# refresh-bio/vclust

Hardware: AMD Instinct MI355X
Metric: genome pairs/sec through prefilter+align (ani.tsv) (higher is better)
Workload: dtype u64

## Files before the change

include/vclust_gpu.h:

```cpp
#ifndef VCLUST_GPU_H
#define VCLUST_GPU_H

#include <stdint.h>

#ifdef __cplusplus
extern "C" {
#endif

enum {
    VG_OK = 0, VG_EINVAL = -1, VG_EIO = -2, VG_ENODEV = -3, VG_EHIP = -4, VG_ENOMEM = -5,
    VG_EOVERFLOW = -6
};

const char* vg_version(void);
const char* vg_last_error(void);
void        vg_free(void* p);
int vg_device_count(void);
int vg_set_device(int device);
void vg_release_device_memory(void);
int vg_alloc_selftest(const int64_t* sizes, int n_sizes, int cycles);
int vg_copy(void* dst, const void* src, int64_t bytes, int to_host);

typedef struct vg_genomes vg_genomes;

// ... 15 lines not shown

int vg_kmer_shared(vg_genomes* g, int k, double fraction, int shard, int n_shards,
                   uint32_t min_shared, int64_t* set_sizes, vg_pair_count** pairs,
                   int64_t* n_pairs);
int vg_kmer_shared_new(vg_genomes* g, int n_db, int k, double fraction, uint32_t min_shared, int64_t* set_sizes,
                       vg_pair_count** pairs, int64_t* n_pairs);
void vg_set_new_path(int mode);
typedef struct {
    int accepted; int64_t P; int n_passes;
    int levels, total_bits, B1, B2;
    int st_tiles; int64_t n_st; int u_st, g_st;
    int tile32k, narrow, short_rec;
} vg_kmer_geometry_info;
int vg_kmer_geometry(const vg_genomes* g, int k, double fraction, int shard, int n_shards, vg_kmer_geometry_info* info);
int vg_kmer_geometry_at(int64_t padded_positions, int k, vg_kmer_geometry_info* info);
int vg_kmer_set(vg_genomes* g, int idx, int k, double fraction, uint64_t** out, int64_t* n_out);

int vg_write_fltr(const vg_genomes* g, int k, double fraction, int min_kmers, double min_ident,
                  int max_seqs, const int64_t* set_sizes, const vg_pair_count* pairs,
                  int64_t n_pairs, const char* out_path);

int vg_filter_pairs(int k, int min_kmers, double min_ident, const int64_t* set_sizes, int64_t n_genomes,
                    const vg_pair_count* pairs, int64_t n_pairs, vg_pair_count** out, int64_t* n_out);

typedef struct {
    int    k;
    int    min_kmers;
    double min_ident;
    int    batch_size;
    double kmers_fraction;
// ... 195 lines not shown
```

vclust_amd/_lib.py:

```python
import ctypes as C
import pathlib

PKG_DIR = pathlib.Path(__file__).resolve().parent
LIB_PATH = PKG_DIR / 'libvclust_gpu.so'


class VclustGpuError(RuntimeError):
    def __init__(self, code, msg):
        super().__init__(f'libvclust_gpu error {code}: {msg}')
        self.code = code


class PairCount(C.Structure):
    _fields_ = [('a', C.c_uint32), ('b', C.c_uint32), ('shared', C.c_uint32)]


class Task(C.Structure):
    _fields_ = [('q', C.c_uint32), ('r', C.c_uint32)]


class PairStat(C.Structure):
    _fields_ = [('n_match', C.c_uint32), ('aln_len', C.c_uint32), ('n_regions', C.c_uint32)]


# ... 96 lines not shown
    'vg_genomes_load': (C.c_int, [P(C.c_char_p), C.c_int, C.c_int, C.c_int, P(C.c_void_p)]),
    'vg_genomes_load_db_new': (C.c_int, [P(C.c_char_p), C.c_int, P(C.c_char_p), C.c_int, C.c_int, C.c_int, P(C.c_void_p), P(C.c_int)]),
    'vg_genomes_from_codes': (C.c_int, [C.c_void_p, C.c_void_p, C.c_int, P(C.c_char_p), P(C.c_void_p)]),
    'vg_genomes_free': (None, [C.c_void_p]),
    'vg_genomes_count': (C.c_int, [C.c_void_p]),
    'vg_genomes_total_len': (C.c_int64, [C.c_void_p]),
    'vg_genomes_lengths': (C.c_int, [C.c_void_p, P(C.c_int64)]),
    'vg_genomes_name': (C.c_char_p, [C.c_void_p, C.c_int]),
    'vg_genomes_codes': (C.c_int, [C.c_void_p, C.c_int, C.c_void_p]),
    'vg_genomes_to_device': (C.c_int, [C.c_void_p]),
    'vg_kmer_shared': (C.c_int, [C.c_void_p, C.c_int, C.c_double, C.c_int, C.c_int, C.c_uint32,
                                 P(C.c_int64), P(P(PairCount)), P(C.c_int64)]),
    'vg_kmer_shared_new': (C.c_int, [C.c_void_p, C.c_int, C.c_int, C.c_double, C.c_uint32, P(C.c_int64), P(P(PairCount)), P(C.c_int64)]),
    'vg_kmer_geometry': (C.c_int, [C.c_void_p, C.c_int, C.c_double, C.c_int, C.c_int, P(KmerGeometry)]),
    'vg_kmer_geometry_at': (C.c_int, [C.c_int64, C.c_int, P(KmerGeometry)]),
    'vg_kmer_set': (C.c_int, [C.c_void_p, C.c_int, C.c_int, C.c_double, P(P(C.c_uint64)), P(C.c_int64)]),
    'vg_filter_pairs': (C.c_int, [C.c_int, C.c_int, C.c_double, C.POINTER(C.c_int64), C.c_int64, C.POINTER(PairCount), C.c_int64,
                                  C.POINTER(C.POINTER(PairCount)), C.POINTER(C.c_int64)]),
    'vg_write_fltr': (C.c_int, [C.c_void_p, C.c_int, C.c_double, C.c_int, C.c_double, C.c_int,
                                P(C.c_int64), P(PairCount), C.c_int64, C.c_char_p]),
    'vg_prefilter': (C.c_int, [P(C.c_char_p), C.c_int, C.c_char_p, P(PrefilterParams)]),
    'vg_prefilter_new': (C.c_int, [P(C.c_char_p), C.c_int, P(C.c_char_p), C.c_int, C.c_char_p, P(PrefilterParams)]),
    'vg_set_process_ends_after_call': (None, [C.c_int]),
    'vg_set_lz_fit': (None, [P(LzFit)]),
    'vg_lz_align': (C.c_int, [C.c_void_p, P(Task), C.c_int64, P(LzParams), P(PairStat),
                              P(P(Region)), P(C.c_int64)]),
    'vg_align_order': (C.c_int, [C.c_void_p, P(C.c_int32)]),
    'vg_read_filter': (C.c_int, [C.c_void_p, C.c_char_p, C.c_double, P(P(PairCount)), P(C.c_int64)]),
    'vg_align_tasks': (C.c_int, [C.c_void_p, P(PairCount), C.c_int64, P(P(Task)), P(C.c_int64)]),
    'vg_lz_prepare': (C.c_int, [C.c_void_p, P(PairCount), C.c_int64, P(LzParams)]),
# ... 98 lines not shown
```

vclust_amd/api.py:

```python
import ctypes as C
import inspect
import os

import numpy as np

from . import _lib
from ._lib import (CLUSTER_ALGORITHMS, LINKAGE_ALGORITHMS, AlignParams, ClusterStats, DedupStats, KernelTime, LinkageStats, LzParams, PairCount, PairStat,
                   PrefilterParams, Region, Task, check)

ALIGN_FIELDS = ['qidx', 'ridx', 'query', 'reference', 'tani', 'gani', 'ani', 'qcov', 'rcov',
                'num_alns', 'len_ratio', 'qlen', 'rlen', 'nt_match', 'nt_mismatch']

PAIR_DTYPE = np.dtype([('a', '<u4'), ('b', '<u4'), ('shared', '<u4')])
TASK_DTYPE = np.dtype([('q', '<u4'), ('r', '<u4')])
STAT_DTYPE = np.dtype([('n_match', '<u4'), ('aln_len', '<u4'), ('n_regions', '<u4')])
REGION_DTYPE = np.dtype([('task', '<u4'), ('qstart', '<i4'), ('qend', '<i4'), ('rstart', '<i4'),
                         ('rend', '<i4'), ('n_match', '<i4')])
LINKAGE_DTYPE = np.dtype([('node_a', '<i8'), ('node_b', '<i8'), ('similarity', '<f8'), ('size', '<i8'), ('object_a', '<i4'),
                          ('object_b', '<i4')])

from .stages import DEFAULT_LZ


def version():
# ... 418 lines not shown

def set_placement_trials(n):
    _lib.load().vg_set_placement_trials(int(n))


def set_new_path(mode):
    _lib.load().vg_set_new_path(int(mode))


def kmer_geometry_at(padded_positions, k=25):
    info = _lib.KmerGeometry()
    check(_lib.load().vg_kmer_geometry_at(int(padded_positions), int(k), C.byref(info)))
    return {name: int(getattr(info, name)) for name, _ in info._fields_}


def release_device_memory():
    _lib.load().vg_release_device_memory()


def profile_enable(on=True):
    _lib.load().vg_profile_enable(int(bool(on)))


def profile_reset():
    _lib.load().vg_profile_reset()


def profile_get():
    lib = _lib.load()
    arr = (KernelTime * 64)()
# ... 4 lines not shown
```

vclust_amd/csrc/vg_prefilter.hip:

```cpp
#include "vg_common.h"
#include <functional>
#include <map>
#include <mutex>
#include <optional>
#include <rocprim/rocprim.hpp>
#include <algorithm>
#include <cmath>
#include <cstring>

namespace {

constexpr uint64_t SENT = ~0ULL;
constexpr uint32_t SCRAMBLE32 = 0x9E3779B1u;
__host__ __device__ __forceinline__ uint64_t scramble_key(uint64_t cano, int k) {
    const uint32_t L = (uint32_t)cano & ((1u << k) - 1u);
    const uint32_t H = (uint32_t)(cano >> k);
    return ((uint64_t)(H ^ ((L * SCRAMBLE32) >> (32 - k))) << k) | L;
}
__host__ __device__ __forceinline__ uint64_t unscramble_key(uint64_t key, int k) { return scramble_key(key, k); }
constexpr uint32_t DUP_BIT = 0x80000000u;

__device__ __forceinline__ uint64_t mix64(uint64_t x) {
    x ^= x >> 33; x *= 0xff51afd7ed558ccdULL; x ^= x >> 33;
    x *= 0xc4ceb9fe1a85ec53ULL; x ^= x >> 33; return x;
}

__device__ __forceinline__ uint64_t rev2(uint64_t x) {
    x = __brevll(x);
    return ((x >> 1) & 0x5555555555555555ULL) | ((x & 0x5555555555555555ULL) << 1);
}

struct kmer_args {
    const uint32_t* planes; const uint32_t* nmask; const uint32_t* blk2g; const int64_t* base_off; const int64_t* len;
    int64_t P; int k; int use_frac; uint64_t frac_thr; uint32_t shard, n_shards; int blk_shift;
    uint32_t dig_lo, dig_n;
// ... 319 lines not shown
            const bool has_next = kk[j + 1] == key;
            const bool dup = has_prev && gg[j - 1] == g;
            gen[i] = g | (dup ? DUP_BIT : 0u);
            if (dup) { atomicAdd(&dup_per_genome[g], 1); continue; }
            if (!has_prev && !has_next) continue;
            if (!has_prev) continue;
            rowinfo[p] = (uint32_t)run_lower(keys, i, key) + 1u;
        }
    }
}

__global__ void __launch_bounds__(256)
k_group_runs(const uint64_t* __restrict__ keys, const uint32_t* __restrict__ pos, const uint32_t* __restrict__ blk2g, int blk_shift,
             int64_t n, int low_bit, uint32_t* __restrict__ gen, uint32_t* __restrict__ rowinfo,
             compact_map M, int* __restrict__ dup_per_genome, int64_t* __restrict__ long_list, unsigned int* __restrict__ n_long,
             unsigned int long_cap) {
    __shared__ uint64_t sk[GS_TILE + GS_HALO + 1];
    __shared__ uint32_t sp[GS_TILE + GS_HALO + 1];
    __shared__ unsigned long long sh[(GS_TILE + GS_HALO + 1) / 64 + 2];
    constexpr int SLOTS = (GS_TILE + GS_HALO + 1 + 255) / 256 * 256;
    const int64_t n_tiles = (n + GS_TILE - 1) / GS_TILE;
    for (int64_t tile = blockIdx.x; tile < n_tiles; tile += gridDim.x) {
        const int64_t t0 = tile * GS_TILE;
        const int m = (int)min<int64_t>((int64_t)GS_TILE + GS_HALO + 1, n - t0 + 1);
        __syncthreads();
        for (int j = threadIdx.x; j < m; j += blockDim.x) {
            const int64_t g = t0 - 1 + j;
            const uint32_t p = g >= 0 ? pos[g] : 0u;
            sk[j] = g >= 0 ? keys[g] : ~0ULL;
            sp[j] = p;
        }
// ... 20 lines not shown
                if (j == gs) { const unsigned int o = atomicAdd(n_long, 1u); if (o < long_cap) long_list[o] = t0 - 1 + gs; }
                continue;
            }
            const uint64_t key = sk[j];
            int lt = 0, eq_before = 0, eq_after = 0, prev_eq = -1;
            for (int t = gs; t < ge; ++t) {
                const uint64_t kt = sk[t];
                lt += kt < key;
                if (kt == key) { if (t < j) { ++eq_before; prev_eq = t; } else if (t > j) ++eq_after; }
            }
            const uint32_t rl = (uint32_t)(eq_before + eq_after + 1);
            if (rl < 2) continue;
            const int64_t rs = t0 - 1 + gs + lt;
            const uint32_t pj = sp[j];
            const uint32_t g = M.cblk ? genome_of_compact(M, pj) : blk2g[pj >> blk_shift];
            bool dup = false;
            if (prev_eq >= 0) { const uint32_t pq = sp[prev_eq]; dup = (M.cblk ? genome_of_compact(M, pq) : blk2g[pq >> blk_shift]) == g; }
            gen[rs + eq_before] = g | (dup ? DUP_BIT : 0u);
            if (dup) { atomicAdd(&dup_per_genome[g], 1); continue; }
            if (eq_before == 0) continue;
            const uint32_t p = sp[j];
            rowinfo[p] = (uint32_t)rs + 1u;
        }
    }
}

__global__ void __launch_bounds__(256)
k_long_groups(const uint64_t* __restrict__ keys, const uint32_t* __restrict__ pos, const uint32_t* __restrict__ blk2g, int blk_shift,
              int64_t n, int low_bit, const int64_t* __restrict__ long_list, uint32_t* __restrict__ gen, uint32_t* __restrict__ rowinfo,
              compact_map M, int* __restrict__ dup_per_genome, unsigned int* __restrict__ need_full_sort) {
    __shared__ int64_t s_end;
    const int64_t gs = long_list[blockIdx.x];
    const uint64_t key0 = keys[gs]; const uint64_t pre = key0 >> low_bit;
    if (threadIdx.x == 0) s_end = n;
    __syncthreads();
    bool same = true;
    for (int64_t base = gs; base < n; base += blockDim.x) {
// ... 35 lines not shown
            uint32_t old = atomicCAS(&hk[h], HT_EMPTY, b);
            if (old == HT_EMPTY) { atomicAdd(n_used, 1u); atomicAdd(&hc[h], 1u); return true; }
            if (old == b) { atomicAdd(&hc[h], 1u); return true; }
        }
        h = (h + 1) & (HT_SIZE - 1);
    }
    return false;
}

template <int HT_BITS, bool COMPACT = false>
__global__ void __launch_bounds__(256)
k_spgemm(const uint32_t* __restrict__ rowinfo, const uint32_t* __restrict__ gen, uint64_t n_gen,
         const int64_t* __restrict__ base_off, const int64_t* __restrict__ len, const uint32_t* __restrict__ wave_base,
         int n_genomes, uint32_t min_emit, const uint32_t* __restrict__ row_list, int n_rows,
         vg_pair_count* __restrict__ out, unsigned long long* __restrict__ out_cursor,
         unsigned long long out_cap, uint32_t* __restrict__ overflow_rows, uint32_t* __restrict__ n_overflow) {
    constexpr int HT_SIZE = 1 << HT_BITS;
    constexpr int ROWS_PER_TRIP = 16;
    __shared__ uint32_t hk[HT_SIZE];
    __shared__ uint32_t hc[HT_SIZE];
    constexpr int LQC = COMPACT ? 64 : LQ_CAP;
    __shared__ uint32_t lq[LQC];
    __shared__ uint32_t rq[COMPACT ? 64 * ROWS_PER_TRIP : 1];
    __shared__ uint32_t s_used, s_lq, s_fail, s_first;
    const int per_xcd = (n_rows + 7) / 8;
    for (int k = (int)(blockIdx.x / 8); k < per_xcd; k += (int)(gridDim.x / 8)) {
    const int row = (int)(blockIdx.x % 8) * per_xcd + k;
    if (row >= n_rows) break;
    const uint32_t a = row_list ? row_list[row] : (uint32_t)row;
    __syncthreads();
    for (int i = threadIdx.x; i < HT_SIZE; i += blockDim.x) { hk[i] = HT_EMPTY; hc[i] = 0; }
    if (threadIdx.x == 0) { s_used = 0; s_lq = 0; s_fail = 0; }
    __syncthreads();
    const int64_t p0 = wave_base ? (int64_t)wave_base[base_off[a] >> 6] : base_off[a];
    const int64_t L = wave_base ? (int64_t)wave_base[base_off[a + 1] >> 6] - p0 : len[a];
    auto walk = [&](uint32_t rs) {
        bool done = false;
        uint32_t e = 0;
        for (; e < (uint32_t)LONG_RUN && !done; e += 4) {
            uint32_t g4[4];
            __builtin_memcpy(g4, gen + (size_t)rs + e, 16);
#pragma unroll
            for (int j = 0; j < 4; ++j) {
                if (done) continue;
                const uint32_t g = g4[j];
                if (g & DUP_BIT) continue;
                if (g >= a) { done = true; continue; }
                if (!ht_add<HT_BITS>(hk, hc, g, &s_used)) s_fail = 1;
            }
        }
        if (!done) {
            const uint32_t slot = atomicAdd(&s_lq, 1u);
            if (slot < LQC) lq[slot] = rs + e;
            else for (uint64_t x = (uint64_t)rs + e; x < n_gen; ++x) {
                const uint32_t g = gen[x];
                if (g & DUP_BIT) continue;
                if (g >= a) break;
                if (!ht_add<HT_BITS>(hk, hc, g, &s_used)) s_fail = 1;
            }
        }
    };
    for (int64_t base = 0; base < L; base += (int64_t)blockDim.x * ROWS_PER_TRIP) {
        uint32_t rr4[ROWS_PER_TRIP];
#pragma unroll
        for (int u = 0; u < ROWS_PER_TRIP; ++u) {
            const int64_t i = base + (int64_t)u * blockDim.x + threadIdx.x;
            rr4[u] = (i < L) ? rowinfo[p0 + i] : 0u;
        }
        if (COMPACT) {
            const int lane = threadIdx.x & 63;
            uint32_t nq = 0;
#pragma unroll
            for (int u = 0; u < ROWS_PER_TRIP; ++u) {
                const bool nz = rr4[u] != 0u;
                const unsigned long long b = __ballot(nz);
                if (nz) rq[nq + (uint32_t)__popcll(b & ((1ULL << lane) - 1ULL))] = rr4[u];
                nq += (uint32_t)__popcll(b);
            }
            __syncthreads();
            for (uint32_t qi = (uint32_t)lane; qi < nq; qi += 64u) walk(rq[qi] - 1u);
        } else {
#pragma unroll
        for (int u = 0; u < ROWS_PER_TRIP; ++u) {
            if (!rr4[u]) continue;
            walk(rr4[u] - 1u);
        }
        }
        __syncthreads();
        if (s_lq >= LQC / 2 || base + (int64_t)blockDim.x * ROWS_PER_TRIP >= L) {
            const uint32_t nq = s_lq < LQC ? s_lq : LQC;
            for (uint32_t qi = 0; qi < nq; ++qi) {
                for (uint64_t c0 = lq[qi]; ; c0 += blockDim.x) {
                    if (threadIdx.x == 0) s_first = 0xffffffffu;
                    __syncthreads();
                    const uint64_t x = c0 + threadIdx.x;
                    const uint32_t g = x < n_gen ? gen[x] : 0u;
                    const bool stop = x >= n_gen || (!(g & DUP_BIT) && g >= a);
                    if (stop) atomicMin(&s_first, (uint32_t)threadIdx.x);
                    __syncthreads();
                    const uint32_t f = s_first;
// ... 22 lines not shown
    __syncthreads();
    if (mine) {
        unsigned long long o = ((unsigned long long)lq[1] << 32 | lq[0]) + at;
        for (int i = threadIdx.x; i < HT_SIZE; i += blockDim.x) {
            const uint32_t b = hk[i];
            if (b != HT_EMPTY && hc[i] >= min_emit) { if (o < out_cap) { out[o].a = a; out[o].b = b; out[o].shared = hc[i]; } ++o; }
        }
    }
    }
}

__global__ void __launch_bounds__(256)
k_spgemm_dense(const uint32_t* __restrict__ rowinfo, const uint32_t* __restrict__ gen, uint64_t n_gen,
               const int64_t* __restrict__ base_off, const int64_t* __restrict__ len, const uint32_t* __restrict__ wave_base,
               int n_genomes, uint32_t min_emit, const uint32_t* __restrict__ rows, uint32_t* __restrict__ dense ,
               vg_pair_count* __restrict__ out, unsigned long long* __restrict__ out_cursor, unsigned long long out_cap) {
    const uint32_t a = rows[blockIdx.x];
    uint32_t* cnt = dense + (size_t)blockIdx.x * n_genomes;
    const int64_t p0 = wave_base ? (int64_t)wave_base[base_off[a] >> 6] : base_off[a];
    const int64_t L = wave_base ? (int64_t)wave_base[base_off[a + 1] >> 6] - p0 : len[a];
    for (int64_t i = threadIdx.x; i < L; i += blockDim.x) {
        const uint32_t r = rowinfo[p0 + i];
        if (!r) continue;
        for (uint64_t x = (uint64_t)r - 1; x < n_gen; ++x) {
            const uint32_t g = gen[x];
            if (g & DUP_BIT) continue;
            if (g >= a) break;
            atomicAdd(&cnt[g], 1u);
        }
    }
    __syncthreads();
    for (uint32_t b = threadIdx.x; b < a; b += blockDim.x) {
        uint32_t c = cnt[b];
        if (c >= min_emit && c > 0) {
            unsigned long long o = atomicAdd(out_cursor, 1ULL);
            if (o < out_cap) { out[o].a = a; out[o].b = b; out[o].shared = c; }
        }
    }
// ... 830 lines not shown
        uint32_t acc = run;
        for (int u = 0; u < n_u; ++u) { const uint32_t t = tab[(size_t)u * nb2 + c]; tab[(size_t)u * nb2 + c] = acc; acc += t; }
        run += tot[v];
    }
    if (b1 == nb1 - 1 && threadIdx.x == 0) boff[(size_t)nb1 * nb2] = off1[nb1];
}

constexpr int BK_PER = BK_CAP / BK_THREADS;
constexpr int BK_MAXBIN = 768;
template <bool NARROW, int THREADS, int SUBBITS>
__global__ void __launch_bounds__(THREADS)
k_bucket_runs(const uint32_t* __restrict__ rec, int stride ,
              const uint32_t* __restrict__ boff, int64_t n_buckets, int pbits, const uint32_t* __restrict__ blk2g, int blk_shift,
              uint32_t* __restrict__ gen, uint32_t* __restrict__ rowinfo, compact_map M, int* __restrict__ dup_per_genome,
              const uint32_t* __restrict__ bucket_list ,
              uint32_t* __restrict__ over_list, unsigned int* __restrict__ n_over) {
    constexpr int BK_SUB = 1 << SUBBITS, CAP = THREADS * BK_PER;
    static_assert(CAP <= 8192 && BK_MAXBIN <= 1024, "slot | rank << 13 of the run members");
    __shared__ uint32_t s_big;
    __shared__ uint64_t sk[CAP];
    __shared__ uint32_t sp[NARROW ? 1 : CAP];
    __shared__ uint32_t sgen[CAP];
    __shared__ uint32_t cnt[BK_SUB + 1], start[BK_SUB + 1];
    __shared__ uint32_t s_wave[THREADS / 64];
    const int lane = threadIdx.x & 63, wv = threadIdx.x >> 6;
    for (int64_t it = blockIdx.x; it < n_buckets; it += gridDim.x) {
        const int64_t bk = bucket_list ? (int64_t)bucket_list[it] : it;
        const uint32_t b0 = boff[bk], b1 = boff[bk + 1];
        const uint32_t n_u = b1 - b0;
        if (n_u <= 1) continue;
        if (n_u > (uint32_t)CAP) { if (threadIdx.x == 0) over_list[atomicAdd(n_over, 1u)] = (uint32_t)bk; continue; }
        const int n = (int)n_u;
// ... 85 lines not shown
                for (uint32_t t = s0; t < s1; ++t) {
                    const uint64_t kt = sk[t];
                    lt += kt < kq;
                    if (kt == kq) { ++eq; before += sp[t] < pq; }
                }
            }
            if (eq < 2) continue;
            const uint32_t g = M.cblk ? genome_of_compact(M, pq) : blk2g[pq >> blk_shift];
            sgen[s0 + lt + before] = g;
            if (before) { at[q] = (s0 + lt + before) | (before << 13); gq[q] = g; }
        }
        lds_sync();
#pragma unroll
        for (int q = 0; q < BK_PER; ++q) {
            if (at[q] == 0xffffffffu) continue;
            const uint32_t slot = at[q] & 0x1fffu, g = gq[q];
            if ((sgen[slot - 1] & ~DUP_BIT) == g) { sgen[slot] = g | DUP_BIT; atomicAdd(&dup_per_genome[g], 1); continue; }
            rowinfo[pj[q]] = b0 + (slot - (at[q] >> 13)) + 1u;
        }
        lds_sync();
        for (uint32_t i = 4u * threadIdx.x; i < (uint32_t)n; i += 4u * THREADS) {
            if (i + 4 <= (uint32_t)n) { const uint4 v = make_uint4(sgen[i], sgen[i + 1], sgen[i + 2], sgen[i + 3]); __builtin_memcpy(gen + b0 + i, &v, 16); }
            else for (uint32_t j = i; j < (uint32_t)n; ++j) gen[b0 + j] = sgen[j];
        }
    }
}

constexpr int BB_THREADS = 1024;
constexpr int BB_DIGITS = 12;
__device__ __forceinline__ uint32_t bb_scan_incl_add(uint32_t v, uint32_t* s_w, uint32_t* carry) {
    const int lane = threadIdx.x & 63, wv = threadIdx.x >> 6;
    uint32_t x = v;
#pragma unroll
// ... 18 lines not shown
    __syncthreads();
    uint32_t base = *carry, tot = *carry;
#pragma unroll
    for (int i = 0; i < BB_THREADS / 64; ++i) { const uint32_t t = s_w[i]; if (i < wv) base = max(base, t); tot = max(tot, t); }
    const uint32_t r = max(base, x);
    __syncthreads();
    if (threadIdx.x == 0) *carry = tot;
    __syncthreads();
    return r;
}
__global__ void __launch_bounds__(BB_THREADS)
k_bucket_big(const uint32_t* __restrict__ rec, int stride, const uint32_t* __restrict__ boff, const uint32_t* __restrict__ list,
             const uint64_t* __restrict__ soff , int pbits,
             uint64_t* __restrict__ kA, uint32_t* __restrict__ pA, uint64_t* __restrict__ kB, uint32_t* __restrict__ pB,
             const uint32_t* __restrict__ blk2g, int blk_shift, uint32_t* __restrict__ gen, uint32_t* __restrict__ rowinfo,
             compact_map M, int* __restrict__ dup_per_genome) {
    __shared__ uint32_t hist[BB_DIGITS][256];
    __shared__ uint32_t gbase[256];
    __shared__ uint32_t wcnt[BB_THREADS / 64][256];
    __shared__ uint32_t s_w[BB_THREADS / 64];
    __shared__ uint32_t s_carry_a, s_carry_b;
    const int lane = threadIdx.x & 63, wv = threadIdx.x >> 6;
    const uint32_t bk = list[blockIdx.x];
    const uint32_t b0 = boff[bk];
    const uint32_t n = boff[bk + 1] - b0;
    uint64_t* k0 = kA + soff[blockIdx.x]; uint32_t* p0 = pA + soff[blockIdx.x];
    uint64_t* k1 = kB + soff[blockIdx.x]; uint32_t* p1 = pB + soff[blockIdx.x];
    for (int i = threadIdx.x; i < BB_DIGITS * 256; i += BB_THREADS) (&hist[0][0])[i] = 0;
    __syncthreads();
    for (uint32_t i = threadIdx.x; i < n; i += BB_THREADS) {
        const uint32_t* r = rec + (uint64_t)(b0 + i) * stride;
// ... 68 lines not shown
        }
        const uint32_t s_incl = bb_scan_incl_add(nd, s_w, &s_carry_a);
        const uint32_t rs = bb_scan_incl_max(hd, s_w, &s_carry_b);
        if (i < n) { S[2 * (uint64_t)i] = s_incl | (nd ? 0u : 0x80000000u); S[2 * (uint64_t)i + 1] = rs; }
    }
    __threadfence_block();
    __syncthreads();
    for (uint32_t i = threadIdx.x; i < n; i += BB_THREADS) {
        const uint32_t sv = S[2 * (uint64_t)i], rs = S[2 * (uint64_t)i + 1];
        const uint32_t pos = p0[i];
        const uint32_t g = M.cblk ? genome_of_compact(M, pos) : blk2g[pos >> blk_shift];
        if (sv & 0x80000000u) { atomicAdd(&dup_per_genome[g], 1); continue; }
        const uint32_t base = rs ? (S[2 * (uint64_t)(rs - 1)] & 0x7fffffffu) : 0u;
        const uint32_t rank = (sv & 0x7fffffffu) - 1u - base;
        gen[(uint64_t)b0 + rs + rank] = g;
        if (rank > 0) rowinfo[pos] = b0 + rs + 1u;
    }
}

__global__ void k_bucket_sizes(const uint32_t* __restrict__ boff, const uint32_t* __restrict__ list, int64_t n, uint32_t* __restrict__ sizes) {
    for (int64_t i = (int64_t)blockIdx.x * blockDim.x + threadIdx.x; i < n; i += (int64_t)gridDim.x * blockDim.x) sizes[i] = boff[list[i] + 1] - boff[list[i]];
}

struct max_op { __device__ __host__ uint32_t operator()(uint32_t a, uint32_t b) const { return a > b ? a : b; } };

}

static int g_force_subshards = 0;
static const char* pf_switch(const char* name) { const char* e = vg_dev_getenv(name); return e ? e : ""; }
static const struct {
    bool radix = !strcmp(pf_switch("VG_INDEX_PATH"), "radix");
    bool long_rec = !strcmp(pf_switch("VG_LEVEL1_RECORDS"), "long");
    bool old_scatter = !strcmp(pf_switch("VG_DENSE_SCATTER"), "staged");
    bool range_dense = !strcmp(pf_switch("VG_RANGE_SCATTER"), "dense");
    bool staged2 = !strcmp(pf_switch("VG_LEVEL2_SCATTER"), "staged");
    bool scan_each = !strcmp(pf_switch("VG_SUBSHARD_SCAN"), "each");
    int subshards = atoi(pf_switch("VG_SUBSHARDS"));
    int placement_trials = atoi(pf_switch("VG_PLACEMENT_TRIALS"));
    double workspace_gb = [] { const char* e = getenv("VG_WORKSPACE_GB"); const double v = e ? atof(e) : 0.0; return v > 0.01 ? v : 8.0; }();
} g_sw{};
template <class F> static void with_k(bool k25, F f) { if (k25) f(std::integral_constant<int, 25>{}); else f(std::integral_constant<int, 0>{}); }
constexpr double SUB_PASS_KMERS = 3.6e9, SUB_PASS_START = 3.9e9;

static bool range_shards(int64_t P, double fraction, int n_shards) {
    return n_shards > 1 && n_shards <= 256 && !(fraction < 1.0) && P < (1LL << 32);
}
static bool range_shards(const vg_genomes* g, double fraction, int n_shards) { return range_shards(g->padded_total(), fraction, n_shards); }
static kmer_args shard_kmer_args(int64_t P, int align_shift, int k, double fraction, int shard, int n_shards) {
    const int use_frac = fraction < 1.0;
    kmer_args A{ nullptr, nullptr, nullptr, nullptr, nullptr, P, k, use_frac,
                 use_frac ? (uint64_t)std::ldexp(fraction, 64) : ~0ULL, (uint32_t)shard, (uint32_t)n_shards, align_shift, 0u, 1u << DIG_BITS, 1u << DIG_BITS };
    if (range_shards(P, fraction, n_shards)) {
        A.dig_max = (uint32_t)(((1u << DIG_BITS) + (uint32_t)n_shards - 1u) / (uint32_t)n_shards);
        const uint32_t lo = (uint32_t)(((uint64_t)shard << DIG_BITS) / (uint64_t)n_shards), hi = (uint32_t)(((uint64_t)(shard + 1) << DIG_BITS) / (uint64_t)n_shards);
        A.shard = 0; A.n_shards = 1; A.dig_lo = lo; A.dig_n = hi - lo;
// ... 243 lines not shown
        if (mine.m_off.empty()) { mine.m_off.assign((size_t)W + 1, 0); mine.t_off.assign((size_t)W + 1, 0); }
        if (status != VG_OK) vg_set_error("%s", err.c_str());
        const vg_xpart parts[2] = { { mine.mask.p, mine.m_off.data(), wave_mask, m_roff.data() }, { mine.T.p, mine.t_off.data(), T1s, t_roff.data() } };
        xs->alltoallv(status, parts, 2);
    }
    if (W_total > 0) hipLaunchKernelGGL(k_mask_popc, dim3(grid_for(W_total)), dim3(256), 0, s, (const unsigned long long*)wave_mask, W_total, wave_cnt);
    VG_HIP(hipStreamSynchronize(s));
}

struct kmer_index {
    sorted_index si;
    dbuf<uint32_t> arena;
    dbuf<uint32_t> rowinfo, gen; dbuf<int> d_dups;
    std::vector<int> kept, dups;
    int64_t nv = 0, n_rows_info = 0;
    bool compact_rows = false, rows_from_map = false;
    const uint32_t* wbase = nullptr;
};
struct bucket_geometry {
    bool range, big_buckets, narrow, tile32k, short_rec;
    int total_bits, B1, B2, levels, bin_lo, nb1g, nb1, nb2, st_tiles, n_slabs; int64_t n_st, nbk;
    lvl2_tab L2;
};
static bool bucket_geometry_for(int k, bool dense, const kmer_args& A, int64_t n_src, bucket_geometry& G) {
    G.range = dense && A.dig_n < (1u << DIG_BITS);
    if (g_sw.radix || n_src < (1 << 16) || n_src >= (1LL << 32)) return false;
    const int64_t n_expect = dense && !G.range ? n_src / std::max<uint32_t>(1u, A.n_shards) : n_src;
    if (!bucket_digits(n_expect, &G.total_bits, &G.B1, &G.B2)) return false;
    G.big_buckets = (n_expect >> G.total_bits) > 1024; G.levels = G.total_bits > 11 ? 2 : 1;
    if (G.range && G.B1 > DIG_BITS) return false;
// ... 143 lines not shown
        }
    }
    VG_HIP(hipStreamSynchronize(s));
    vg_host_mark("buckets: level 2 done");
    vg_deferred_start();
    R.f_rec = R.b_rec.p; R.f_stride = G.narrow ? 2 : 3;
    ix.arena = std::move(R.a_rec);
    if (!R.rows_zero.e) ix.rowinfo.view(ix.arena.p, (size_t)ix.n_rows_info);
    ix.gen.view(ix.arena.p + (((size_t)ix.n_rows_info + 3) & ~(size_t)3), (size_t)R.n1 + 4);
}
static void bucket_kernels(bucket_run& R) {
    const bucket_geometry& G = R.G; hipStream_t s = R.s; vg_genomes* g = R.g; kmer_index& ix = R.ix;
    const uint32_t n1 = R.n1; const int64_t nbk = G.nbk;
    if (ix.gen.n < (size_t)n1 + 4) ix.gen.alloc((size_t)n1 + 4);
    if (ix.rowinfo.n < (size_t)ix.n_rows_info) ix.rowinfo.alloc((size_t)ix.n_rows_info);
    dbuf<unsigned int> d_nover(2); d_nover.zero(s);
    dbuf<uint32_t> over1((size_t)nbk), over2;
    if (R.rows_zero.e) VG_HIP(hipStreamWaitEvent(s, R.rows_zero.e, 0));
    else VG_HIP(hipMemsetAsync(ix.rowinfo.p, 0, (size_t)ix.n_rows_info * sizeof(uint32_t), s));
    const int pb = G.narrow ? 0 : G.total_bits;
    const uint32_t* boff = R.boff.p; const uint32_t* blk2g = g->d_blk2g.p;
    unsigned int n_over[2] = {0, 0};
    auto runs = [&](auto kern, int threads, int grid, int64_t count, const uint32_t* list, uint32_t* over, unsigned int* nover) {
        hipLaunchKernelGGL(kern, dim3(grid), dim3(threads), 0, s, R.f_rec, R.f_stride, boff, count, pb, blk2g, g->align_shift, ix.gen.p, ix.rowinfo.p, R.cmap, ix.d_dups.p, list, over, nover);
    };
    const auto wide = G.narrow ? k_bucket_runs<true, 1024, 11> : k_bucket_runs<false, 1024, 11>;
    {
        vg_prof_scope ps("bucket_sort_runs", (double)n1 * ((G.narrow ? 8 : 12) + 4 + 8));
        const int grid_b = (int)std::min<int64_t>(nbk, 256 * 16);
        if (G.big_buckets) runs(wide, 1024, grid_b, nbk, nullptr, over1.p, d_nover.p);
        else runs(G.narrow ? k_bucket_runs<true, BK_THREADS, 9> : k_bucket_runs<false, BK_THREADS, 9>, BK_THREADS, grid_b, nbk, nullptr, over1.p, d_nover.p);
        d_nover.download(n_over, 2, s);
        VG_HIP(hipStreamSynchronize(s));
    }
    const uint32_t* big_list = over1.p; unsigned int n_big = n_over[0];
    if (n_big > 0 && !G.big_buckets) {
        over2.alloc((size_t)n_big);
        vg_prof_scope ps("bucket_sort_runs_wide", 0);
        runs(wide, 1024, (int)std::min<int64_t>(n_big, 256 * 16), n_big, over1.p, over2.p, d_nover.p + 1);
// ... 2 lines not shown
        big_list = over2.p; n_big = n_over[1];
    }
    if (n_big == 0) return;
    dbuf<uint32_t> d_sz(n_big); std::vector<uint32_t> sz(n_big);
    hipLaunchKernelGGL(k_bucket_sizes, dim3(grid_for(n_big)), dim3(256), 0, s, boff, big_list, (int64_t)n_big, d_sz.p);
    d_sz.download(sz.data(), n_big, s);
    VG_HIP(hipStreamSynchronize(s));
    std::vector<uint64_t> so(n_big); uint64_t tot = 0;
    for (unsigned int i = 0; i < n_big; ++i) { so[i] = tot; tot += ((uint64_t)sz[i] + 3) & ~3ULL; }
    dbuf<uint64_t> d_so(n_big);
    d_so.upload(so.data(), n_big, s);
    dbuf<uint64_t> kA((size_t)tot + 4), kB((size_t)tot + 4); dbuf<uint32_t> pA((size_t)tot + 4), pB((size_t)tot + 4);
    {
        vg_prof_scope ps("bucket_big", (double)tot * 12.0 * 2.0);
        hipLaunchKernelGGL(k_bucket_big, dim3(n_big), dim3(BB_THREADS), 0, s, R.f_rec, R.f_stride, boff, big_list,
                           (const uint64_t*)d_so.p, pb, kA.p, pA.p, kB.p, pB.p, blk2g, g->align_shift, ix.gen.p, ix.rowinfo.p, R.cmap, ix.d_dups.p);
    }
    VG_HIP(hipStreamSynchronize(s));
}
static bool start_bucket_run(bucket_run& R, const kmer_args& A) {
    const bool dense = R.dense; const int k = R.k; kmer_index& ix = R.ix;
    R.rows_zero.st = R.s;
    const int64_t n_src = dense ? R.g->padded_total() : ix.nv;
    if (!bucket_geometry_for(k, dense, A, n_src, R.G)) return false;
    const bucket_geometry& G = R.G;
    R.S.A = A; R.S.keys = dense ? nullptr : ix.si.keys.p; R.S.pos = dense ? nullptr : ix.si.pos.p; R.S.n = n_src; R.S.k2 = 2 * k; R.S.bin_lo = G.bin_lo;
    R.cmap = dense ? compact_map{ nullptr, nullptr } : compact_map{ ix.si.goff.p, ix.si.cblk.p };
    R.k25 = dense && k == 25 && !A.use_frac && A.n_shards == 1;
    R.T1s.alloc((size_t)G.nb1 * (size_t)G.n_st + 1); R.slab.alloc((size_t)G.n_slabs * G.nb1); R.d_off1.alloc((size_t)G.nb1 + 1);
    R.G.L2.T1s = R.T1s.p; R.G.L2.off1 = R.d_off1.p;
    return true;
// ... 43 lines not shown
}
static void index_by_radix(vg_genomes* g, int k, double fraction, int shard, int n_shards, const pass_inputs& in, kmer_index& ix) {
    hipStream_t s = vg_stream(); const int n = g->n;
    sorted_index& si = ix.si; dbuf<uint32_t>& rowinfo = ix.rowinfo; dbuf<uint32_t>& gen = ix.gen; dbuf<int>& d_dups = ix.d_dups;
    rowinfo.release(); gen.release(); ix.arena.release();
    d_dups.zero(s);
    si = sorted_index();
    run_extract_sort(g, k, fraction, shard, n_shards, in, si, false);
    const int64_t nv = ix.nv = si.n_valid;
    ix.n_rows_info = si.compact ? std::max<int64_t>(nv, 1) : g->padded_total();
    if (2 * si.spare64.n >= (size_t)ix.n_rows_info) rowinfo.view(reinterpret_cast<uint32_t*>(si.spare64.p), (size_t)ix.n_rows_info);
    else rowinfo.alloc((size_t)ix.n_rows_info);
    VG_HIP(hipMemsetAsync(rowinfo.p, 0, (size_t)ix.n_rows_info * sizeof(uint32_t), s));
    const compact_map cmap{ si.compact ? si.goff.p : nullptr, si.compact ? si.cblk.p : nullptr };
    gen = si.spare32.n >= (size_t)std::max<int64_t>(nv, 1) + 4 ? std::move(si.spare32) : dbuf<uint32_t>((size_t)std::max<int64_t>(nv, 1) + 4);
    constexpr unsigned int LONG_CAP = 1u << 16;
    dbuf<int64_t> long_list(LONG_CAP); dbuf<unsigned int> d_nlong(1), d_full(1); d_nlong.zero(s); d_full.zero(s);
    if (nv > 0) {
        vg_prof_scope ps("index_runs", (double)nv * (8 + 4 + 4 + 8));
        hipLaunchKernelGGL(k_group_runs, dim3(grid_for(nv, GS_TILE)), dim3(256), 0, s, si.keys.p, si.pos.p, g->d_blk2g.p, g->align_shift, nv,
                           si.low_bit, gen.p, rowinfo.p, cmap, d_dups.p, long_list.p, d_nlong.p, LONG_CAP);
    }
    unsigned int n_long = 0, need_full = 0;
    d_nlong.download(&n_long, 1, s); si.kept.download(ix.kept.data(), (size_t)n, s); d_dups.download(ix.dups.data(), (size_t)n, s);
    VG_HIP(hipStreamSynchronize(s));
    if (n_long > 0 && n_long <= LONG_CAP) {
        {
            vg_prof_scope ps("index_long_runs", 0);
            hipLaunchKernelGGL(k_long_groups, dim3(n_long), dim3(256), 0, s, si.keys.p, si.pos.p, g->d_blk2g.p, g->align_shift, nv, si.low_bit,
                               long_list.p, gen.p, rowinfo.p, cmap, d_dups.p, d_full.p);
        }
        d_full.download(&need_full, 1, s); d_dups.download(ix.dups.data(), (size_t)n, s);
        VG_HIP(hipStreamSynchronize(s));
    }
    if (need_full || n_long > LONG_CAP) {
        rowinfo.zero(s); d_dups.zero(s);
// ... 28 lines not shown
            if (n_large) { d_large.alloc(large_rows.size()); d_large.upload(large_rows.data(), large_rows.size(), s); }
        }
    }
    dbuf<uint32_t> d_tail;
    if (first_row > 0 && !n_small) {
        std::vector<uint32_t> tail((size_t)(n - first_row));
        for (int i = first_row; i < n; ++i) tail[(size_t)(i - first_row)] = (uint32_t)i;
        d_tail.alloc(tail.size()); d_tail.upload(tail.data(), tail.size(), s);
        VG_HIP(hipStreamSynchronize(s));
    }
    for (;;) {
        dbuf<vg_pair_count> d_out((size_t)cap);
        d_cursor.zero(s); d_nover.zero(s);
        auto launch = [&](auto kern, int threads, const uint32_t* rows, int n_rows, uint32_t* over) {
            hipLaunchKernelGGL(kern, dim3((n_rows + 7) / 8 * 8), dim3(threads), 0, s, ix.rowinfo.p, ix.gen.p, (uint64_t)ix.gen.n, g->d_base_off.p, g->d_len.p, ix.wbase, n,
                               min_shared, rows, n_rows, d_out.p, d_cursor.p, cap, over, d_nover.p);
        };
        {
            vg_prof_scope ps("spgemm_rows", (double)ix.n_rows_info * 4.0);
            if (n_small) {
                if (n_large) launch(k_spgemm<11>, 256, d_large.p, n_large, d_over.p);
                launch(k_spgemm<9, true>, 64, d_small.p, n_small, d_over.p);
            } else launch(k_spgemm<11>, 256, d_tail.p, n - first_row, d_over.p);
        }
        constexpr size_t EAGER = 1 << 16;
        uint32_t nover = 0; unsigned long long produced = 0;
        host_pairs.resize(dev_out ? 0 : std::min<size_t>(EAGER, (size_t)cap));
        d_nover.download(&nover, 1, s); d_cursor.download(&produced, 1, s);
        if (!dev_out) d_out.download(host_pairs.data(), host_pairs.size(), s);
        VG_HIP(hipStreamSynchronize(s));
        vg_host_mark("spgemm done");
// ... 8 lines not shown
            }
            VG_HIP(hipMemcpyAsync(d_over.p, d_over2.p, sizeof(uint32_t) * nover, hipMemcpyDeviceToDevice, s));
            d_nover.download(&nover, 1, s);
            VG_HIP(hipStreamSynchronize(s));
        }
        if (nover > 0) {
            std::vector<uint32_t> rows(nover); d_over.download(rows.data(), nover, s); VG_HIP(hipStreamSynchronize(s));
            const uint32_t batch = (uint32_t)std::max<int64_t>(1, std::min<int64_t>(nover, (int64_t)(1u << 28) / std::max(n, 1)));
            dbuf<uint32_t> dense((size_t)batch * n), d_rows(batch);
            for (uint32_t o = 0; o < nover; o += batch) {
                uint32_t nb = std::min(batch, nover - o);
                dense.zero(s);
                d_rows.upload(rows.data() + o, nb, s);
                vg_prof_scope ps("spgemm_dense_rows", 0);
                hipLaunchKernelGGL(k_spgemm_dense, dim3(nb), dim3(256), 0, s, ix.rowinfo.p, ix.gen.p, (uint64_t)ix.gen.n, g->d_base_off.p,
                                   g->d_len.p, ix.wbase, n, min_shared, d_rows.p, dense.p, d_out.p, d_cursor.p, cap);
                VG_HIP(hipStreamSynchronize(s));
            }
        }
        d_cursor.download(&produced, 1, s);
        VG_HIP(hipStreamSynchronize(s));
        if (produced <= cap) {
            if (dev_out) { *dev_out = std::move(d_out); *dev_n = produced; break; }
            host_pairs.resize((size_t)produced);
            if (produced) d_out.download(host_pairs.data(), (size_t)produced, s);
            VG_HIP(hipStreamSynchronize(s));
            break;
        }
        cap = produced + produced / 8 + 1024;
    }
}
// ... 425 lines not shown
    const bool masked = subshards_share_scan(g, fraction, n_shards, plan.sub);
    const bool dense = pass_source_dense(P, fraction, ns, masked);
    report_geometry(k, dense, shard_kmer_args(P, g->align_shift, k, 1.0, sh, ns), P, info);
    VG_API_END
}
extern "C" int vg_kmer_geometry_at(int64_t padded_positions, int k, vg_kmer_geometry_info* info) {
    VG_API_BEGIN
    if (!info) throw vg_error(VG_EINVAL, "vg_kmer_geometry_at: null argument");
    if (k < 8 || k > 31) throw vg_error(VG_EINVAL, "k out of range (8..31)");
    if (padded_positions < 0) throw vg_error(VG_EINVAL, "vg_kmer_geometry_at: negative number of positions");
    memset(info, 0, sizeof *info);
    info->P = padded_positions; info->n_passes = 1;
    report_geometry(k, true, shard_kmer_args(padded_positions, 0, k, 1.0, 0, 1), padded_positions, info);
    VG_API_END
}

extern "C" int vg_kmer_set(vg_genomes* g, int idx, int k, double fraction, uint64_t** out, int64_t* n_out) {
    VG_API_BEGIN
    if (!g || !out || !n_out || idx < 0 || idx >= g->n) throw vg_error(VG_EINVAL, "vg_kmer_set: bad argument");
    if (k < 8 || k > 31) throw vg_error(VG_EINVAL, "k out of range (8..31)");
    vg_require_device();
    int rc = vg_genomes_to_device(g); if (rc) return rc;
    hipStream_t s = vg_stream();
    sorted_index si;
    run_extract_sort(g, k, fraction, 0, 1, pass_inputs{}, si);
    std::vector<uint64_t> keys((size_t)si.n_valid); std::vector<uint32_t> pos((size_t)si.n_valid);
    if (si.n_valid) { si.keys.download(keys.data(), keys.size(), s); si.pos.download(pos.data(), pos.size(), s); }
    VG_HIP(hipStreamSynchronize(s));
    std::vector<uint64_t> mine;
    int64_t lo = g->base_off[idx], hi = g->base_off[idx + 1];
// ... 26 lines not shown
```

Baseline: 2.600 million.

## Inline single-partner rowptr entries as genome ids to skip gen walks

When a k-mer position has exactly one earlier distinct genome in its run, rowinfo now stores an encoded genome id (from the top of the uint32 range) instead of a pointer into gen. The SpGEMM kernels detect these inline values and add the partner straight into the hash table or dense counter, avoiding a dependent global load and walk. The sparse path also prefetches the first four gen entries for a batch of rows before walking, to overlap loads. Inlining is disabled when the entry count would collide with the reserved range, and it can be switched off with VG_ROWPTR_INLINE=0.

Result: no change. 2.652 million (median of 6 runs) (+2.0%).

```diff
diff --git a/include/vclust_gpu.h b/include/vclust_gpu.h
--- a/include/vclust_gpu.h
+++ b/include/vclust_gpu.h
@@ -53,6 +53,7 @@
 } vg_kmer_geometry_info;
 int vg_kmer_geometry(const vg_genomes* g, int k, double fraction, int shard, int n_shards, vg_kmer_geometry_info* info);
 int vg_kmer_geometry_at(int64_t padded_positions, int k, vg_kmer_geometry_info* info);
+int vg_rowptr_inline_lo(int64_t entries, int64_t n_genomes, uint32_t* inline_lo);
 int vg_kmer_set(vg_genomes* g, int idx, int k, double fraction, uint64_t** out, int64_t* n_out);
 
 int vg_write_fltr(const vg_genomes* g, int k, double fraction, int min_kmers, double min_ident,
diff --git a/vclust_amd/_lib.py b/vclust_amd/_lib.py
--- a/vclust_amd/_lib.py
+++ b/vclust_amd/_lib.py
@@ -134,6 +134,7 @@
     'vg_kmer_shared_new': (C.c_int, [C.c_void_p, C.c_int, C.c_int, C.c_double, C.c_uint32, P(C.c_int64), P(P(PairCount)), P(C.c_int64)]),
     'vg_kmer_geometry': (C.c_int, [C.c_void_p, C.c_int, C.c_double, C.c_int, C.c_int, P(KmerGeometry)]),
     'vg_kmer_geometry_at': (C.c_int, [C.c_int64, C.c_int, P(KmerGeometry)]),
+    'vg_rowptr_inline_lo': (C.c_int, [C.c_int64, C.c_int64, P(C.c_uint32)]),
     'vg_kmer_set': (C.c_int, [C.c_void_p, C.c_int, C.c_int, C.c_double, P(P(C.c_uint64)), P(C.c_int64)]),
     'vg_filter_pairs': (C.c_int, [C.c_int, C.c_int, C.c_double, C.POINTER(C.c_int64), C.c_int64, C.POINTER(PairCount), C.c_int64,
                                   C.POINTER(C.POINTER(PairCount)), C.POINTER(C.c_int64)]),
diff --git a/vclust_amd/api.py b/vclust_amd/api.py
--- a/vclust_amd/api.py
+++ b/vclust_amd/api.py
@@ -456,6 +456,12 @@
     return {name: int(getattr(info, name)) for name, _ in info._fields_}
 
 
+def rowptr_inline_lo(entries, n_genomes):
+    lo = C.c_uint32(0)
+    check(_lib.load().vg_rowptr_inline_lo(int(entries), int(n_genomes), C.byref(lo)))
+    return int(lo.value)
+
+
 def release_device_memory():
     _lib.load().vg_release_device_memory()
 
diff --git a/vclust_amd/csrc/vg_prefilter.hip b/vclust_amd/csrc/vg_prefilter.hip
--- a/vclust_amd/csrc/vg_prefilter.hip
+++ b/vclust_amd/csrc/vg_prefilter.hip
@@ -19,6 +19,8 @@
 }
 __host__ __device__ __forceinline__ uint64_t unscramble_key(uint64_t key, int k) { return scramble_key(key, k); }
 constexpr uint32_t DUP_BIT = 0x80000000u;
+__device__ __forceinline__ uint32_t rowptr_inline(uint32_t partner) { return 0xFFFFFFFFu - partner; }
+__device__ __forceinline__ uint32_t rowptr_partner_of_rs(uint32_t rs) { return 0xFFFFFFFEu - rs; }
 
 __device__ __forceinline__ uint64_t mix64(uint64_t x) {
     x ^= x >> 33; x *= 0xff51afd7ed558ccdULL; x ^= x >> 33;
@@ -368,7 +370,7 @@
 k_group_runs(const uint64_t* __restrict__ keys, const uint32_t* __restrict__ pos, const uint32_t* __restrict__ blk2g, int blk_shift,
              int64_t n, int low_bit, uint32_t* __restrict__ gen, uint32_t* __restrict__ rowinfo,
              compact_map M, int* __restrict__ dup_per_genome, int64_t* __restrict__ long_list, unsigned int* __restrict__ n_long,
-             unsigned int long_cap) {
+             unsigned int long_cap, uint32_t inline_lo) {
     __shared__ uint64_t sk[GS_TILE + GS_HALO + 1];
     __shared__ uint32_t sp[GS_TILE + GS_HALO + 1];
     __shared__ unsigned long long sh[(GS_TILE + GS_HALO + 1) / 64 + 2];
@@ -419,13 +421,13 @@
             const int64_t rs = t0 - 1 + gs + lt;
             const uint32_t pj = sp[j];
             const uint32_t g = M.cblk ? genome_of_compact(M, pj) : blk2g[pj >> blk_shift];
-            bool dup = false;
-            if (prev_eq >= 0) { const uint32_t pq = sp[prev_eq]; dup = (M.cblk ? genome_of_compact(M, pq) : blk2g[pq >> blk_shift]) == g; }
+            bool dup = false; uint32_t g_prev = 0;
+            if (prev_eq >= 0) { const uint32_t pq = sp[prev_eq]; g_prev = M.cblk ? genome_of_compact(M, pq) : blk2g[pq >> blk_shift]; dup = g_prev == g; }
             gen[rs + eq_before] = g | (dup ? DUP_BIT : 0u);
             if (dup) { atomicAdd(&dup_per_genome[g], 1); continue; }
             if (eq_before == 0) continue;
             const uint32_t p = sp[j];
-            rowinfo[p] = (uint32_t)rs + 1u;
+            rowinfo[p] = (inline_lo && eq_before == 1) ? rowptr_inline(g_prev) : (uint32_t)rs + 1u;
         }
     }
 }
@@ -491,8 +493,9 @@
          const int64_t* __restrict__ base_off, const int64_t* __restrict__ len, const uint32_t* __restrict__ wave_base,
          int n_genomes, uint32_t min_emit, const uint32_t* __restrict__ row_list, int n_rows,
          vg_pair_count* __restrict__ out, unsigned long long* __restrict__ out_cursor,
-         unsigned long long out_cap, uint32_t* __restrict__ overflow_rows, uint32_t* __restrict__ n_overflow) {
+         unsigned long long out_cap, uint32_t* __restrict__ overflow_rows, uint32_t* __restrict__ n_overflow, uint32_t inline_lo) {
     constexpr int HT_SIZE = 1 << HT_BITS;
+    const uint32_t inl = inline_lo - 1u;
     constexpr int ROWS_PER_TRIP = 16;
     __shared__ uint32_t hk[HT_SIZE];
     __shared__ uint32_t hc[HT_SIZE];
@@ -511,20 +514,24 @@
     __syncthreads();
     const int64_t p0 = wave_base ? (int64_t)wave_base[base_off[a] >> 6] : base_off[a];
     const int64_t L = wave_base ? (int64_t)wave_base[base_off[a + 1] >> 6] - p0 : len[a];
-    auto walk = [&](uint32_t rs) {
+    auto take4 = [&](const uint32_t* g4, bool& done) {
+#pragma unroll
+        for (int j = 0; j < 4; ++j) {
+            if (done) continue;
+            const uint32_t g = g4[j];
+            if (g & DUP_BIT) continue;
+            if (g >= a) { done = true; continue; }
+            if (!ht_add<HT_BITS>(hk, hc, g, &s_used)) s_fail = 1;
+        }
+    };
+    auto walk = [&](uint32_t rs, const uint32_t* first = nullptr ) {
         bool done = false;
         uint32_t e = 0;
+        if (first) { take4(first, done); e = 4; }
         for (; e < (uint32_t)LONG_RUN && !done; e += 4) {
             uint32_t g4[4];
             __builtin_memcpy(g4, gen + (size_t)rs + e, 16);
-#pragma unroll
-            for (int j = 0; j < 4; ++j) {
-                if (done) continue;
-                const uint32_t g = g4[j];
-                if (g & DUP_BIT) continue;
-                if (g >= a) { done = true; continue; }
-                if (!ht_add<HT_BITS>(hk, hc, g, &s_used)) s_fail = 1;
-            }
+            take4(g4, done);
         }
         if (!done) {
             const uint32_t slot = atomicAdd(&s_lq, 1u);
@@ -549,18 +556,32 @@
             uint32_t nq = 0;
 #pragma unroll
             for (int u = 0; u < ROWS_PER_TRIP; ++u) {
-                const bool nz = rr4[u] != 0u;
+                const bool il = rr4[u] != 0u && rr4[u] - 1u >= inl;
+                const bool nz = rr4[u] != 0u && !il;
                 const unsigned long long b = __ballot(nz);
                 if (nz) rq[nq + (uint32_t)__popcll(b & ((1ULL << lane) - 1ULL))] = rr4[u];
                 nq += (uint32_t)__popcll(b);
+                if (il && !ht_add<HT_BITS>(hk, hc, rowptr_partner_of_rs(rr4[u] - 1u), &s_used)) s_fail = 1;
             }
             __syncthreads();
             for (uint32_t qi = (uint32_t)lane; qi < nq; qi += 64u) walk(rq[qi] - 1u);
         } else {
-#pragma unroll
-        for (int u = 0; u < ROWS_PER_TRIP; ++u) {
-            if (!rr4[u]) continue;
-            walk(rr4[u] - 1u);
+        constexpr int HB = 8;
+#pragma unroll
+        for (int h = 0; h < ROWS_PER_TRIP; h += HB) {
+            uint32_t f[HB][4];
+#pragma unroll
+            for (int u = 0; u < HB; ++u) {
+                f[u][0] = f[u][1] = f[u][2] = f[u][3] = 0u;
+                if (rr4[h + u] != 0u && rr4[h + u] - 1u < inl) __builtin_memcpy(f[u], gen + (size_t)(rr4[h + u] - 1u), 16);
+            }
+#pragma unroll
+            for (int u = 0; u < HB; ++u) {
+                if (!rr4[h + u]) continue;
+                const uint32_t rs = rr4[h + u] - 1u;
+                if (rs >= inl) { if (!ht_add<HT_BITS>(hk, hc, rowptr_partner_of_rs(rs), &s_used)) s_fail = 1; continue; }
+                walk(rs, f[u]);
+            }
         }
         }
         __syncthreads();
@@ -613,14 +634,16 @@
 k_spgemm_dense(const uint32_t* __restrict__ rowinfo, const uint32_t* __restrict__ gen, uint64_t n_gen,
                const int64_t* __restrict__ base_off, const int64_t* __restrict__ len, const uint32_t* __restrict__ wave_base,
                int n_genomes, uint32_t min_emit, const uint32_t* __restrict__ rows, uint32_t* __restrict__ dense ,
-               vg_pair_count* __restrict__ out, unsigned long long* __restrict__ out_cursor, unsigned long long out_cap) {
+               vg_pair_count* __restrict__ out, unsigned long long* __restrict__ out_cursor, unsigned long long out_cap, uint32_t inline_lo) {
     const uint32_t a = rows[blockIdx.x];
+    const uint32_t inl = inline_lo - 1u;
     uint32_t* cnt = dense + (size_t)blockIdx.x * n_genomes;
     const int64_t p0 = wave_base ? (int64_t)wave_base[base_off[a] >> 6] : base_off[a];
     const int64_t L = wave_base ? (int64_t)wave_base[base_off[a + 1] >> 6] - p0 : len[a];
     for (int64_t i = threadIdx.x; i < L; i += blockDim.x) {
         const uint32_t r = rowinfo[p0 + i];
         if (!r) continue;
+        if (r - 1u >= inl) { atomicAdd(&cnt[rowptr_partner_of_rs(r - 1u)], 1u); continue; }
         for (uint64_t x = (uint64_t)r - 1; x < n_gen; ++x) {
             const uint32_t g = gen[x];
             if (g & DUP_BIT) continue;
@@ -1481,8 +1504,9 @@
               const uint32_t* __restrict__ boff, int64_t n_buckets, int pbits, const uint32_t* __restrict__ blk2g, int blk_shift,
               uint32_t* __restrict__ gen, uint32_t* __restrict__ rowinfo, compact_map M, int* __restrict__ dup_per_genome,
               const uint32_t* __restrict__ bucket_list ,
-              uint32_t* __restrict__ over_list, unsigned int* __restrict__ n_over) {
+              uint32_t* __restrict__ over_list, unsigned int* __restrict__ n_over, uint32_t inline_lo) {
     constexpr int BK_SUB = 1 << SUBBITS, CAP = THREADS * BK_PER;
+    const uint32_t inline_rank = inline_lo ? 1u : 0u;
     static_assert(CAP <= 8192 && BK_MAXBIN <= 1024, "slot | rank << 13 of the run members");
     __shared__ uint32_t s_big;
     __shared__ uint64_t sk[CAP];
@@ -1598,9 +1622,10 @@
 #pragma unroll
         for (int q = 0; q < BK_PER; ++q) {
             if (at[q] == 0xffffffffu) continue;
-            const uint32_t slot = at[q] & 0x1fffu, g = gq[q];
-            if ((sgen[slot - 1] & ~DUP_BIT) == g) { sgen[slot] = g | DUP_BIT; atomicAdd(&dup_per_genome[g], 1); continue; }
-            rowinfo[pj[q]] = b0 + (slot - (at[q] >> 13)) + 1u;
+            const uint32_t slot = at[q] & 0x1fffu, g = gq[q], before = at[q] >> 13;
+            const uint32_t g_prev = sgen[slot - 1] & ~DUP_BIT;
+            if (g_prev == g) { sgen[slot] = g | DUP_BIT; atomicAdd(&dup_per_genome[g], 1); continue; }
+            rowinfo[pj[q]] = before == inline_rank ? rowptr_inline(g_prev) : b0 + (slot - before) + 1u;
         }
         lds_sync();
         for (uint32_t i = 4u * threadIdx.x; i < (uint32_t)n; i += 4u * THREADS) {
@@ -1649,7 +1674,7 @@
              const uint64_t* __restrict__ soff , int pbits,
              uint64_t* __restrict__ kA, uint32_t* __restrict__ pA, uint64_t* __restrict__ kB, uint32_t* __restrict__ pB,
              const uint32_t* __restrict__ blk2g, int blk_shift, uint32_t* __restrict__ gen, uint32_t* __restrict__ rowinfo,
-             compact_map M, int* __restrict__ dup_per_genome) {
+             compact_map M, int* __restrict__ dup_per_genome, uint32_t inline_lo) {
     __shared__ uint32_t hist[BB_DIGITS][256];
     __shared__ uint32_t gbase[256];
     __shared__ uint32_t wcnt[BB_THREADS / 64][256];
@@ -1748,7 +1773,13 @@
         const uint32_t base = rs ? (S[2 * (uint64_t)(rs - 1)] & 0x7fffffffu) : 0u;
         const uint32_t rank = (sv & 0x7fffffffu) - 1u - base;
         gen[(uint64_t)b0 + rs + rank] = g;
-        if (rank > 0) rowinfo[pos] = b0 + rs + 1u;
+        if (rank == 0) continue;
+        uint32_t v = b0 + rs + 1u;
+        if (inline_lo && rank == 1u) {
+            const uint32_t pf = p0[rs];
+            v = rowptr_inline(M.cblk ? genome_of_compact(M, pf) : blk2g[pf >> blk_shift]);
+        }
+        rowinfo[pos] = v;
     }
 }
 
@@ -1769,10 +1800,16 @@
     bool range_dense = !strcmp(pf_switch("VG_RANGE_SCATTER"), "dense");
     bool staged2 = !strcmp(pf_switch("VG_LEVEL2_SCATTER"), "staged");
     bool scan_each = !strcmp(pf_switch("VG_SUBSHARD_SCAN"), "each");
+    bool no_inline = !strcmp(pf_switch("VG_ROWPTR_INLINE"), "0");
     int subshards = atoi(pf_switch("VG_SUBSHARDS"));
     int placement_trials = atoi(pf_switch("VG_PLACEMENT_TRIALS"));
     double workspace_gb = [] { const char* e = getenv("VG_WORKSPACE_GB"); const double v = e ? atof(e) : 0.0; return v > 0.01 ? v : 8.0; }();
 } g_sw{};
+static uint32_t rowptr_inline_lo(uint64_t entries, int64_t n_genomes) {
+    if (g_sw.no_inline || n_genomes < 1 || entries >= (1ULL << 32) || (uint64_t)n_genomes >= (1ULL << 32)) return 0u;
+    const uint64_t lo = (1ULL << 32) - (uint64_t)n_genomes;
+    return entries < lo ? (uint32_t)lo : 0u;
+}
 template <class F> static void with_k(bool k25, F f) { if (k25) f(std::integral_constant<int, 25>{}); else f(std::integral_constant<int, 0>{}); }
 constexpr double SUB_PASS_KMERS = 3.6e9, SUB_PASS_START = 3.9e9;
 
@@ -2046,6 +2083,7 @@
     dbuf<uint32_t> rowinfo, gen; dbuf<int> d_dups;
     std::vector<int> kept, dups;
     int64_t nv = 0, n_rows_info = 0;
+    uint32_t inline_lo = 0;
     bool compact_rows = false, rows_from_map = false;
     const uint32_t* wbase = nullptr;
 };
@@ -2219,6 +2257,7 @@
     const uint32_t n1 = R.n1; const int64_t nbk = G.nbk;
     if (ix.gen.n < (size_t)n1 + 4) ix.gen.alloc((size_t)n1 + 4);
     if (ix.rowinfo.n < (size_t)ix.n_rows_info) ix.rowinfo.alloc((size_t)ix.n_rows_info);
+    ix.inline_lo = rowptr_inline_lo((uint64_t)ix.gen.n, g->n);
     dbuf<unsigned int> d_nover(2); d_nover.zero(s);
     dbuf<uint32_t> over1((size_t)nbk), over2;
     if (R.rows_zero.e) VG_HIP(hipStreamWaitEvent(s, R.rows_zero.e, 0));
@@ -2227,7 +2266,7 @@
     const uint32_t* boff = R.boff.p; const uint32_t* blk2g = g->d_blk2g.p;
     unsigned int n_over[2] = {0, 0};
     auto runs = [&](auto kern, int threads, int grid, int64_t count, const uint32_t* list, uint32_t* over, unsigned int* nover) {
-        hipLaunchKernelGGL(kern, dim3(grid), dim3(threads), 0, s, R.f_rec, R.f_stride, boff, count, pb, blk2g, g->align_shift, ix.gen.p, ix.rowinfo.p, R.cmap, ix.d_dups.p, list, over, nover);
+        hipLaunchKernelGGL(kern, dim3(grid), dim3(threads), 0, s, R.f_rec, R.f_stride, boff, count, pb, blk2g, g->align_shift, ix.gen.p, ix.rowinfo.p, R.cmap, ix.d_dups.p, list, over, nover, ix.inline_lo);
     };
     const auto wide = G.narrow ? k_bucket_runs<true, 1024, 11> : k_bucket_runs<false, 1024, 11>;
     {
@@ -2260,7 +2299,7 @@
     {
         vg_prof_scope ps("bucket_big", (double)tot * 12.0 * 2.0);
         hipLaunchKernelGGL(k_bucket_big, dim3(n_big), dim3(BB_THREADS), 0, s, R.f_rec, R.f_stride, boff, big_list,
-                           (const uint64_t*)d_so.p, pb, kA.p, pA.p, kB.p, pB.p, blk2g, g->align_shift, ix.gen.p, ix.rowinfo.p, R.cmap, ix.d_dups.p);
+                           (const uint64_t*)d_so.p, pb, kA.p, pA.p, kB.p, pB.p, blk2g, g->align_shift, ix.gen.p, ix.rowinfo.p, R.cmap, ix.d_dups.p, ix.inline_lo);
     }
     VG_HIP(hipStreamSynchronize(s));
 }
@@ -2334,12 +2373,13 @@
     VG_HIP(hipMemsetAsync(rowinfo.p, 0, (size_t)ix.n_rows_info * sizeof(uint32_t), s));
     const compact_map cmap{ si.compact ? si.goff.p : nullptr, si.compact ? si.cblk.p : nullptr };
     gen = si.spare32.n >= (size_t)std::max<int64_t>(nv, 1) + 4 ? std::move(si.spare32) : dbuf<uint32_t>((size_t)std::max<int64_t>(nv, 1) + 4);
+    ix.inline_lo = rowptr_inline_lo((uint64_t)gen.n, n);
     constexpr unsigned int LONG_CAP = 1u << 16;
     dbuf<int64_t> long_list(LONG_CAP); dbuf<unsigned int> d_nlong(1), d_full(1); d_nlong.zero(s); d_full.zero(s);
     if (nv > 0) {
         vg_prof_scope ps("index_runs", (double)nv * (8 + 4 + 4 + 8));
         hipLaunchKernelGGL(k_group_runs, dim3(grid_for(nv, GS_TILE)), dim3(256), 0, s, si.keys.p, si.pos.p, g->d_blk2g.p, g->align_shift, nv,
-                           si.low_bit, gen.p, rowinfo.p, cmap, d_dups.p, long_list.p, d_nlong.p, LONG_CAP);
+                           si.low_bit, gen.p, rowinfo.p, cmap, d_dups.p, long_list.p, d_nlong.p, LONG_CAP, ix.inline_lo);
     }
     unsigned int n_long = 0, need_full = 0;
     d_nlong.download(&n_long, 1, s); si.kept.download(ix.kept.data(), (size_t)n, s); d_dups.download(ix.dups.data(), (size_t)n, s);
@@ -2398,7 +2438,7 @@
         d_cursor.zero(s); d_nover.zero(s);
         auto launch = [&](auto kern, int threads, const uint32_t* rows, int n_rows, uint32_t* over) {
             hipLaunchKernelGGL(kern, dim3((n_rows + 7) / 8 * 8), dim3(threads), 0, s, ix.rowinfo.p, ix.gen.p, (uint64_t)ix.gen.n, g->d_base_off.p, g->d_len.p, ix.wbase, n,
-                               min_shared, rows, n_rows, d_out.p, d_cursor.p, cap, over, d_nover.p);
+                               min_shared, rows, n_rows, d_out.p, d_cursor.p, cap, over, d_nover.p, ix.inline_lo);
         };
         {
             vg_prof_scope ps("spgemm_rows", (double)ix.n_rows_info * 4.0);
@@ -2437,7 +2477,7 @@
                 d_rows.upload(rows.data() + o, nb, s);
                 vg_prof_scope ps("spgemm_dense_rows", 0);
                 hipLaunchKernelGGL(k_spgemm_dense, dim3(nb), dim3(256), 0, s, ix.rowinfo.p, ix.gen.p, (uint64_t)ix.gen.n, g->d_base_off.p,
-                                   g->d_len.p, ix.wbase, n, min_shared, d_rows.p, dense.p, d_out.p, d_cursor.p, cap);
+                                   g->d_len.p, ix.wbase, n, min_shared, d_rows.p, dense.p, d_out.p, d_cursor.p, cap, ix.inline_lo);
                 VG_HIP(hipStreamSynchronize(s));
             }
         }
@@ -2893,6 +2933,13 @@
     report_geometry(k, true, shard_kmer_args(padded_positions, 0, k, 1.0, 0, 1), padded_positions, info);
     VG_API_END
 }
+extern "C" int vg_rowptr_inline_lo(int64_t entries, int64_t n_genomes, uint32_t* inline_lo) {
+    VG_API_BEGIN
+    if (!inline_lo) throw vg_error(VG_EINVAL, "vg_rowptr_inline_lo: null argument");
+    if (entries < 0 || n_genomes < 0) throw vg_error(VG_EINVAL, "vg_rowptr_inline_lo: negative count");
+    *inline_lo = rowptr_inline_lo((uint64_t)entries, n_genomes);
+    VG_API_END
+}
 
 extern "C" int vg_kmer_set(vg_genomes* g, int idx, int k, double fraction, uint64_t** out, int64_t* n_out) {
     VG_API_BEGIN
```
